# ilpoviertola/V-AURA

Hardware: AMD Instinct MI355X
Metric: audio codec tokens/sec (whole node), 2.56 s clips (higher is better)
Workload: dtype f16x2-split(22b)/f32-acc

## Files before the change

### vaura_amd/csrc/conv_kernels.h

```cpp
#pragma once
#include "common.h"

#define BM 128
#define BN 96
#define BK 32

struct ConvArgs {
  const float* in;
  const float* w;
  const float* bias;
  const float* res;
  const float* alpha;
  float* out_raw;
  float* out_act;
  int Lin, Lout, Cin, Cout, NT;
  int off_base, off_step;
  int ostride, oshift0;
  int jcount;
};

__host__ __device__ __forceinline__ size_t mx8_scale_offset(size_t elems) { return (elems + 15) & ~(size_t)15; }

__device__ __forceinline__ float snake_sin2(float x) {
  const float n = __builtin_rintf(x * 0.318309886183790672f);
  float r = fmaf(-n, 3.14159274101257324f, x);
  r = fmaf(-n, -8.74227765734758577e-8f, r);
  const float t = r * r;
  float p = fmaf(t, 2.6051661734527443e-06f, -0.00019809046352747828f);
  p = fmaf(t, p, 0.008333050645887852f);
  p = fmaf(t, p, -0.16666658222675323f);
  const float sn = fmaf(r, t * p, r);
  return sn * sn;
}
__device__ __forceinline__ float snake_fi(float v, float al, float inv) { return v + inv * snake_sin2(al * v); }
__device__ __forceinline__ float snake_f(float v, float al) { return snake_fi(v, al, 1.0f / (al + 1e-9f)); }

typedef _Float16 f16x8 __attribute__((ext_vector_type(8)));

struct ConvPArgs {
  const uint16_t* in;
  const uint16_t* w;
  const float* bias;
  const float* res;
  const float* alpha;
  float* out_raw;
  uint16_t* out_act;
  int Lin, Lout, Cin, Cout, NT;
  int off_base, off_step, ostride, oshift0, jcount;
  int act;
  int act_fmt;
  uint8_t* out_scale;
  const uint32_t* in_scale;
  const float* wscale;
  const uint16_t* w2;
  const float* bias2;
  const float* alpha_mid;
};

template <class Args>
static inline int va_conv_geometry(Args& a, int taps, int dilation, int stride, int Lin) {
  if (stride > 1) {
    a.NT = 2; a.off_base = 0; a.off_step = -1; a.ostride = stride; a.oshift0 = -(stride / 2);
    a.Lout = Lin * stride; a.jcount = Lin + 1;
    return stride;
  }
  a.NT = taps; a.off_base = -((taps - 1) / 2) * dilation; a.off_step = dilation;
  a.ostride = 1; a.oshift0 = 0; a.Lout = Lin; a.jcount = Lin;
  return 1;
}

int va_launch_conv_pair_tile(const ConvPArgs& p, int B, hipStream_t s);

__device__ __forceinline__ float gelu_erf_f(float x) {
  const float t = fabsf(x) * 0.70710678118654752440f;
  const float k = __builtin_amdgcn_rcpf(fmaf(t, 0.35f, 1.0f));
  float p = 0.06797561794519424f;
  p = fmaf(p, k, -0.4044332206249237f);
  p = fmaf(p, k, 0.8392713069915771f);
  p = fmaf(p, k, -0.7225478887557983f);
  p = fmaf(p, k, 0.6403822898864746f);
  p = fmaf(p, k, -0.046077974140644073f);
  p = fmaf(p, k, 0.23748238384723663f);
  p = fmaf(p, k, 0.1900186985731125f);
  p = fmaf(p, k, 0.1979287713766098f);
  const float e = (k * p) * __builtin_amdgcn_exp2f(-(t * t) * 1.4426950408889634f);
  return (0.5f * x) * (x < 0.f ? e : 2.0f - e);
}

__device__ __forceinline__ void store_pair4(uint16_t* base, size_t row, int c0, int C, const f32x4 v) {
  _Float16 h[4], l[4];
#pragma unroll
  for (int i = 0; i < 4; ++i) {
    const float x = v[i];
    h[i] = (_Float16)x;
    l[i] = (_Float16)(x - (float)h[i]);
  }
  typedef _Float16 f16x4 __attribute__((ext_vector_type(4)));
  f16x4* p = reinterpret_cast<f16x4*>(base + ((row * (size_t)(C >> 3) + (size_t)(c0 >> 3)) * 2) * 8 + (c0 & 7));
  p[0] = f16x4{h[0], h[1], h[2], h[3]};
  p[2] = f16x4{l[0], l[1], l[2], l[3]};
}

__device__ __forceinline__ int mx8_scale_byte(float amax) {
  const uint32_t bits = __builtin_bit_cast(uint32_t, amax);
  const int ea = (int)((bits >> 23) & 0xffu);
  const int e8 = ea - ((bits & 0x7fffffu) <= 0x600000u ? 8 : 7);
  return e8 < 1 ? 1 : (e8 > 253 ? 253 : e8);
}

__device__ __forceinline__ void store_act_octet(void* out_act, uint8_t* out_scale, int fmt, size_t grow, int co, int C,
                                                const float (&sv)[8]) {
  if (fmt == 0) {
    f16x8 hi, lo;
#pragma unroll
    for (int r = 0; r < 8; ++r) { hi[r] = (_Float16)sv[r]; lo[r] = (_Float16)(sv[r] - (float)hi[r]); }
    f16x8* dst = reinterpret_cast<f16x8*>(reinterpret_cast<uint16_t*>(out_act) + ((grow * (size_t)(C >> 3) + (size_t)(co >> 3)) * 2) * 8);
    dst[0] = hi;
    dst[1] = lo;
  } else {
    float amax = 0.f;
#pragma unroll
    for (int r = 0; r < 8; ++r) amax = fmaxf(amax, fabsf(sv[r]));
    amax = fmaxf(amax, __shfl_xor(amax, 1, 64));
    amax = fmaxf(amax, __shfl_xor(amax, 2, 64));
    const int e8 = mx8_scale_byte(amax);
    const float inv = __builtin_bit_cast(float, (uint32_t)(254 - e8) << 23);
    int q0 = 0, q1 = 0;
    q0 = __builtin_amdgcn_cvt_pk_fp8_f32(sv[0] * inv, sv[1] * inv, q0, false);
    q0 = __builtin_amdgcn_cvt_pk_fp8_f32(sv[2] * inv, sv[3] * inv, q0, true);
    q1 = __builtin_amdgcn_cvt_pk_fp8_f32(sv[4] * inv, sv[5] * inv, q1, false);
    q1 = __builtin_amdgcn_cvt_pk_fp8_f32(sv[6] * inv, sv[7] * inv, q1, true);
    typedef int i32x2 __attribute__((ext_vector_type(2)));
    *reinterpret_cast<i32x2*>(reinterpret_cast<uint8_t*>(out_act) + grow * (size_t)C + co) = i32x2{q0, q1};
    if (((co >> 3) & 3) == 0) out_scale[(grow * (size_t)((C + 127) >> 7) + (co >> 7)) * 4 + ((co >> 5) & 3)] = (uint8_t)e8;
  }
}

__device__ __forceinline__ float snake_fast(float v, float al) {
  const float sn = __builtin_amdgcn_sinf(__builtin_amdgcn_fractf(al * v * 0.15915494309189535f));
  return v + __builtin_amdgcn_rcpf(al + 1e-9f) * (sn * sn);
}

template <int BN_, int SP, bool FAST = false, int ROWS = BM>
__device__ __forceinline__ void conv_tile_store(const ConvPArgs& a, const float* stage, int b, int ph, int j0, int n0, int tid) {
  constexpr int OCT = BN_ / 8;
  static_assert(OCT % 4 == 0, "a 32-channel scale block = 4 consecutive threads of one row");
  constexpr int RSTEP = 256 / OCT;
  if (tid >= RSTEP * OCT) return;
  const int oc = tid % OCT, row0 = tid / OCT;
  const int co = n0 + oc * 8;
  const size_t obase = (size_t)b * a.Lout;
  f32x4 al0 = f32x4{0.f, 0.f, 0.f, 0.f}, al1 = al0, iv0 = al0, iv1 = al0;
  if (a.out_act && a.act == 0) {
    al0 = *reinterpret_cast<const f32x4*>(a.alpha + co);
    al1 = *reinterpret_cast<const f32x4*>(a.alpha + co + 4);
// ... 37 lines not shown
```

### vaura_amd/csrc/dac.hip

```cpp
#include "conv_kernels.h"
#include "dac_clips.h"

__global__ __launch_bounds__(256) void conv_mfma_kernel(ConvArgs a) {
  __shared__ f32x4 Ws[2][BK / 4][BN + 1];
  __shared__ f32x4 Xs[2][BK / 4][BM + 1];
  const int tid = threadIdx.x, lane = tid & 63, wv = tid >> 6;
  const int wn = wv & 1, wm = wv >> 1;
  const int j0 = blockIdx.x * BM;
  const int n0 = blockIdx.y * BN;
  const int tiles_m = gridDim.x;
  (void)tiles_m;
  const int phases = a.ostride;
  const int b = blockIdx.z / phases, ph = blockIdx.z % phases;
  const float* in = a.in + (size_t)b * a.Lin * a.Cin;
  const float* wbase = a.w + (size_t)ph * a.NT * a.Cout * a.Cin;
  const int kc = a.Cin / BK;
  const int nk = a.NT * kc;

  f32x4 wreg[3], xreg[4];
  auto load_tile = [&](int kt) {
    const int t = kt / kc, ci0 = (kt % kc) * BK;
    const float* wt = wbase + (size_t)t * a.Cout * a.Cin;
    const int off = a.off_base + t * a.off_step;
#pragma unroll
    for (int i = 0; i < 3; ++i) {
      const int qd = tid + 256 * i, row = qd >> 3, kq = qd & 7;
      wreg[i] = *reinterpret_cast<const f32x4*>(wt + (size_t)(n0 + row) * a.Cin + ci0 + 4 * kq);
    }
#pragma unroll
    for (int i = 0; i < 4; ++i) {
      const int qd = tid + 256 * i, row = qd >> 3, kq = qd & 7;
      const int jr = j0 + row + off;
      xreg[i] = (jr >= 0 && jr < a.Lin) ? *reinterpret_cast<const f32x4*>(in + (size_t)jr * a.Cin + ci0 + 4 * kq)
                                        : f32x4{0.f, 0.f, 0.f, 0.f};
    }
  };
  auto store_tile = [&](int buf) {
#pragma unroll
    for (int i = 0; i < 3; ++i) { const int qd = tid + 256 * i; Ws[buf][qd & 7][qd >> 3] = wreg[i]; }
#pragma unroll
    for (int i = 0; i < 4; ++i) { const int qd = tid + 256 * i; Xs[buf][qd & 7][qd >> 3] = xreg[i]; }
  };

  f32x4 acc[3][4];
#pragma unroll
  for (int i = 0; i < 3; ++i)
#pragma unroll
    for (int j = 0; j < 4; ++j) acc[i][j] = f32x4{0.f, 0.f, 0.f, 0.f};

  load_tile(0);
  store_tile(0);
  __syncthreads();
  for (int kt = 0; kt < nk; ++kt) {
    const int buf = kt & 1;
    if (kt + 1 < nk) load_tile(kt + 1);
#pragma unroll
    for (int c = 0; c < 2; ++c) {
      f32x4 af[3], bf[4];
#pragma unroll
      for (int i = 0; i < 3; ++i) af[i] = Ws[buf][4 * c + (lane >> 4)][wn * 48 + i * 16 + (lane & 15)];
#pragma unroll
      for (int j = 0; j < 4; ++j) bf[j] = Xs[buf][4 * c + (lane >> 4)][wm * 64 + j * 16 + (lane & 15)];
#pragma unroll
      for (int s = 0; s < 4; ++s)
#pragma unroll
        for (int i = 0; i < 3; ++i)
#pragma unroll
          for (int j = 0; j < 4; ++j)
            acc[i][j] = __builtin_amdgcn_mfma_f32_16x16x4f32(af[i][s], bf[j][s], acc[i][j], 0, 0, 0);
    }
    if (kt + 1 < nk) store_tile(buf ^ 1);
    __syncthreads();
  }

  const size_t obase = (size_t)b * a.Lout * a.Cout;
#pragma unroll
  for (int j = 0; j < 4; ++j) {
    const int jr = j0 + wm * 64 + j * 16 + (lane & 15);
    if (jr >= a.jcount) continue;
    const int orow = jr * a.ostride + a.oshift0 + ph;
    if (orow < 0 || orow >= a.Lout) continue;
#pragma unroll
    for (int i = 0; i < 3; ++i) {
      const int co = n0 + wn * 48 + i * 16 + 4 * (lane >> 4);
      const size_t o = obase + (size_t)orow * a.Cout + co;
      f32x4 v = acc[i][j] + *reinterpret_cast<const f32x4*>(a.bias + co);
      if (a.res) v = *reinterpret_cast<const f32x4*>(a.res + o) + v;
      if (a.out_raw) *reinterpret_cast<f32x4*>(a.out_raw + o) = v;
      if (a.out_act) {
        const f32x4 al = *reinterpret_cast<const f32x4*>(a.alpha + co);
        f32x4 s;
#pragma unroll
        for (int r = 0; r < 4; ++r) s[r] = snake_f(v[r], al[r]);
        *reinterpret_cast<f32x4*>(a.out_act + o) = s;
      }
    }
  }
}

#define XHALO 56
#define XROWS (BM + XHALO)
template <int NI, bool WS, bool XS = false, int MJ = 4, bool FUSE = false>
__global__ __launch_bounds__(256, 2) void conv_pair_kernel(ConvPArgs a) {
  constexpr int BN_ = 32 * NI;
  constexpr int BMT = 32 * MJ;
  constexpr int XROWS_T = BMT + XHALO;
  constexpr int NXB = MJ == 4 ? 2 : 1;
  static_assert(MJ == 4 || MJ == 8, "128 or 256 rows");
  constexpr int WSTR = (BN_ + 3 + 15) / 16 * 16, XSTR = (XROWS_T + 3 + 15) / 16 * 16;
  constexpr int WS_ELEMS = 2 * (BK / 4) * WSTR, XS_ELEMS = NXB * (BK / 4) * XSTR;
  constexpr int SP = BN_ + 4;
  static_assert((WS_ELEMS + XS_ELEMS) * 16 >= BM * SP * 4, "the output tile must fit in the main loop's LDS");
  static_assert(!FUSE || (NI == 3 && MJ == 8), "the fused residual unit: all 96 channels in one 256-row workgroup");
  constexpr int W1STR = 112, YSTR = 80;
  constexpr int W1_ELEMS = FUSE ? 3 * (BK / 4) * W1STR : 0, Y_ELEMS = FUSE ? 3 * (BK / 4) * YSTR : 0;
  static_assert(!FUSE || Y_ELEMS * 16 >= 64 * SP * 4, "the 64-row output tile is staged over the activated tile");
  constexpr int SMEM_ELEMS = (WS_ELEMS + XS_ELEMS) > (W1_ELEMS + Y_ELEMS) ? (WS_ELEMS + XS_ELEMS) : (W1_ELEMS + Y_ELEMS);
  constexpr int TAB_ELEMS = FUSE ? 2 * BN_ / 4 : 0;
  __shared__ u32x4 smem[SMEM_ELEMS + TAB_ELEMS];
  auto coff = [](int kq) { return (kq & 1) + ((kq >> 2) << 1); };
  auto Ws = [&](int buf, int kq, int row) -> u32x4& { return smem[(buf * (BK / 4) + kq) * WSTR + row + coff(kq)]; };
  auto Xs = [&](int buf, int kq, int row) -> u32x4& { return smem[WS_ELEMS + (buf * (BK / 4) + kq) * XSTR + row + coff(kq)]; };
  const int tid = threadIdx.x, lane = tid & 63, wv = tid >> 6;
  const int wn = wv & 1, wm = wv >> 1;
  const int j0 = blockIdx.x * BMT;
  const int n0 = blockIdx.y * BN_;
  const int phases = a.ostride;
  const int b = blockIdx.z / phases, ph = blockIdx.z % phases;
  const int cq = a.Cin / 4;
  const u32x4* in = reinterpret_cast<const u32x4*>(a.in) + (size_t)b * a.Lin * cq;
  const u32x4* wbase = reinterpret_cast<const u32x4*>(a.w) + (size_t)ph * a.NT * a.Cout * cq;
  const int kc = a.Cin / BK;
  const int NT = a.NT;
  const int nk = NT * kc;
  const int span = (NT - 1) * (a.off_step < 0 ? -a.off_step : a.off_step);
  const int lo_off = a.off_base + (a.off_step < 0 ? (NT - 1) * a.off_step : 0);
  const int xrows = BMT + span;
  constexpr int XL = (XROWS_T * (BK / 4) + 255) / 256;

  u32x4 wreg[NI], xreg[XL];
  auto load_w = [&](int kt) {
    const int c = kt / NT, t = kt - c * NT;
    const u32x4* wt = wbase + (size_t)t * a.Cout * cq;
    const int q0 = c * (BK / 4);
#pragma unroll
    for (int i = 0; i < NI; ++i) {
      const int qd = tid + 256 * i, row = qd >> 3, kq = qd & 7;
      wreg[i] = wt[(size_t)(n0 + row) * cq + q0 + kq];
    }
  };
  auto store_w = [&](int buf) {
#pragma unroll
    for (int i = 0; i < NI; ++i) { const int qd = tid + 256 * i; Ws(buf, qd & 7, qd >> 3) = wreg[i]; }
  };
  auto load_x = [&](int c) {
    const int q0 = c * (BK / 4);
#pragma unroll
    for (int i = 0; i < XL; ++i) {
      const int qd = tid + 256 * i, row = qd >> 3, kq = qd & 7;
      const int jr = j0 + lo_off + row;
      xreg[i] = (row < xrows && jr >= 0 && jr < a.Lin) ? in[(size_t)jr * cq + q0 + kq] : u32x4{0u, 0u, 0u, 0u};
    }
  };
  auto store_x = [&](int buf) {
#pragma unroll
    for (int i = 0; i < XL; ++i) {
      const int qd = tid + 256 * i;
      if ((qd >> 3) < XROWS_T) Xs(buf, qd & 7, qd >> 3) = xreg[i];
    }
  };

  f32x4 acc[NI][MJ];
#pragma unroll
  for (int i = 0; i < NI; ++i)
#pragma unroll
    for (int j = 0; j < MJ; ++j) acc[i][j] = f32x4{0.f, 0.f, 0.f, 0.f};

  VA_STAMP_DECL(stamps);
  VA_STAMP(stamps, 0);
  load_w(0);
  load_x(0);
  store_w(0);
  store_x(0);
  if constexpr (FUSE) {
    if (tid < BN_) {
      float* tab = reinterpret_cast<float*>(smem + SMEM_ELEMS);
      const float al = a.alpha_mid[tid];
      tab[tid] = al;
      tab[BN_ + tid] = 1.0f / (al + 1e-9f);
    }
  }
  __syncthreads();
  VA_STAMP(stamps, 1);
  const int g = lane >> 4, r16 = lane & 15;
  int kt = 0;
  for (int c = 0; c < kc; ++c) {
    const int xb = NXB == 2 ? (c & 1) : 0;
    for (int t = 0; t < NT; ++t, ++kt) {
      const int buf = kt & 1;
      if (kt + 1 < nk) load_w(kt + 1);
      if (t == (NXB == 2 ? 0 : NT - 1) && c + 1 < kc) load_x(c + 1);
      const int shift = a.off_base + t * a.off_step - lo_off;
      f16x8 wh[NI], wl[NI];
#pragma unroll
      for (int i = 0; i < NI; ++i) {
        wh[i] = __builtin_bit_cast(f16x8, Ws(buf, 2 * g, wn * (NI * 16) + i * 16 + r16));
        if constexpr (!WS && !XS) wl[i] = __builtin_bit_cast(f16x8, Ws(buf, 2 * g + 1, wn * (NI * 16) + i * 16 + r16));
      }
      constexpr int JG = MJ == 4 ? 4 : 2;
#pragma unroll
      for (int jh = 0; jh < MJ; jh += JG) {
        f16x8 xh[JG], xl[JG];
#pragma unroll
        for (int j = 0; j < JG; ++j) {
          xh[j] = __builtin_bit_cast(f16x8, Xs(xb, 2 * g, shift + wm * (16 * MJ) + (jh + j) * 16 + r16));
          if constexpr (!XS) xl[j] = __builtin_bit_cast(f16x8, Xs(xb, 2 * g + 1, shift + wm * (16 * MJ) + (jh + j) * 16 + r16));
        }
#pragma unroll
        for (int i = 0; i < NI; ++i)
#pragma unroll
          for (int j = 0; j < JG; ++j) {
            if constexpr (!WS && !XS) acc[i][jh + j] = __builtin_amdgcn_mfma_f32_16x16x32_f16(wl[i], xh[j], acc[i][jh + j], 0, 0, 0);
            if constexpr (!XS) acc[i][jh + j] = __builtin_amdgcn_mfma_f32_16x16x32_f16(wh[i], xl[j], acc[i][jh + j], 0, 0, 0);
            acc[i][jh + j] = __builtin_amdgcn_mfma_f32_16x16x32_f16(wh[i], xh[j], acc[i][jh + j], 0, 0, 0);
          }
      }
      if (kt + 1 < nk) store_w(buf ^ 1);
      if (t == NT - 1 && c + 1 < kc) {
        if constexpr (NXB == 1) __syncthreads();
        store_x(NXB == 2 ? (xb ^ 1) : 0);
      }
      __syncthreads();
    }
  }

  VA_STAMP(stamps, 2);
  if constexpr (FUSE) {
    u32x4* W1 = smem;
    u32x4* Yi = smem + W1_ELEMS;
    auto W1s = [&](int c2, int kq, int row) -> u32x4& { return W1[(c2 * (BK / 4) + kq) * W1STR + row + coff(kq)]; };
    auto Ys = [&](int c2, int kq, int row) -> u32x4& { return Yi[(c2 * (BK / 4) + kq) * YSTR + row + coff(kq)]; };
    u32x4 w1reg[9];
#pragma unroll
    for (int i = 0; i < 9; ++i) w1reg[i] = reinterpret_cast<const u32x4*>(a.w2)[tid + 256 * i];
    float* stage = reinterpret_cast<float*>(Yi);
    const float* tab = reinterpret_cast<const float*>(smem + SMEM_ELEMS);
    typedef _Float16 f16x4 __attribute__((ext_vector_type(4)));
    auto pass = [&](auto pc) {
      constexpr int p = decltype(pc)::value;
      if (p > 0) __syncthreads();
      if (wm == (p >> 1)) {
#pragma unroll
        for (int jj = 0; jj < 4; ++jj)
#pragma unroll
          for (int i = 0; i < NI; ++i) {
            const int col = wn * (NI * 16) + i * 16 + 4 * g;
            const f32x4 v = acc[i][4 * (p & 1) + jj] + *reinterpret_cast<const f32x4*>(a.bias + col);
            const f32x4 al = *reinterpret_cast<const f32x4*>(tab + col), iv = *reinterpret_cast<const f32x4*>(tab + BN_ + col);
            f16x4 h4, l4;
#pragma unroll
            for (int e = 0; e < 4; ++e) {
              const float sv = snake_fi(v[e], al[e], iv[e]);
              h4[e] = (_Float16)sv;
              l4[e] = (_Float16)(sv - (float)h4[e]);
            }
            const int c2 = col >> 5, o = (col & 31) >> 3, half = (col & 7) >> 2, row = jj * 16 + r16;
            reinterpret_cast<f16x4*>(&Ys(c2, 2 * o, row))[half] = h4;
            reinterpret_cast<f16x4*>(&Ys(c2, 2 * o + 1, row))[half] = l4;
          }
      }
      if (p == 0) {
#pragma unroll
        for (int i = 0; i < 9; ++i) {
          const int qd = tid + 256 * i, n = qd / 24, q = qd - n * 24;
          W1s(q >> 3, q & 7, n) = w1reg[i];
        }
      }
      __syncthreads();
      if (p == 0) VA_STAMP(stamps, 3);
      f32x4 acc2[NI][2];
#pragma unroll
      for (int i = 0; i < NI; ++i)
#pragma unroll
        for (int j = 0; j < 2; ++j) acc2[i][j] = f32x4{0.f, 0.f, 0.f, 0.f};
#pragma unroll
      for (int c2 = 0; c2 < 3; ++c2) {
        f16x8 wh[NI], wl[NI], xh[2], xl[2];
#pragma unroll
        for (int i = 0; i < NI; ++i) {
          wh[i] = __builtin_bit_cast(f16x8, W1s(c2, 2 * g, wn * (NI * 16) + i * 16 + r16));
          if constexpr (!WS && !XS) wl[i] = __builtin_bit_cast(f16x8, W1s(c2, 2 * g + 1, wn * (NI * 16) + i * 16 + r16));
        }
#pragma unroll
        for (int j = 0; j < 2; ++j) {
          xh[j] = __builtin_bit_cast(f16x8, Ys(c2, 2 * g, (wm * 2 + j) * 16 + r16));
          if constexpr (!XS) xl[j] = __builtin_bit_cast(f16x8, Ys(c2, 2 * g + 1, (wm * 2 + j) * 16 + r16));
        }
#pragma unroll
        for (int i = 0; i < NI; ++i)
#pragma unroll
          for (int j = 0; j < 2; ++j) {
            if constexpr (!WS && !XS) acc2[i][j] = __builtin_amdgcn_mfma_f32_16x16x32_f16(wl[i], xh[j], acc2[i][j], 0, 0, 0);
            if constexpr (!XS) acc2[i][j] = __builtin_amdgcn_mfma_f32_16x16x32_f16(wh[i], xl[j], acc2[i][j], 0, 0, 0);
            acc2[i][j] = __builtin_amdgcn_mfma_f32_16x16x32_f16(wh[i], xh[j], acc2[i][j], 0, 0, 0);
          }
      }
      __syncthreads();
      if (p == 0) VA_STAMP(stamps, 4);
#pragma unroll
      for (int i = 0; i < NI; ++i)
#pragma unroll
        for (int j = 0; j < 2; ++j) {
          const int row = (wm * 2 + j) * 16 + r16, col = wn * (NI * 16) + i * 16 + 4 * g;
          *reinterpret_cast<f32x4*>(stage + row * SP + col) = acc2[i][j] + *reinterpret_cast<const f32x4*>(a.bias2 + col);
        }
      __syncthreads();
// ... 484 lines not shown
  d += __shfl_xor(d, 1, 64);
  d += __shfl_xor(d, 2, 64);
  d += __shfl_xor(d, 4, 64);
  if (sub == 0 && l < L) wav[(size_t)b * L + l] = tanhf(d + bias[0]);
}

#define CO_TL 128
__global__ __launch_bounds__(256) void conv_out_tiled_kernel(const float* __restrict__ act, const float* __restrict__ w,
                                                              const float* __restrict__ bias, float* __restrict__ wav, int L, int C,
                                                              int pairs) {
  extern __shared__ __attribute__((aligned(16))) float rows[];
  const int b = blockIdx.y, l0 = blockIdx.x * CO_TL, tid = threadIdx.x;
  const int SR = C + 4, oct = C >> 3;
  for (int u = tid; u < (CO_TL + 6) * oct; u += 256) {
    const int rr = u / oct, oc = u - rr * oct;
    const int r = l0 - 3 + rr;
    float x[8];
    if (r < 0 || r >= L) {
#pragma unroll
      for (int e = 0; e < 8; ++e) x[e] = 0.f;
    } else if (pairs == 3) {
      const uint8_t* q = reinterpret_cast<const uint8_t*>(act) + (size_t)b * L * C;
      const int nsc = (C + 127) >> 7;
      const uint8_t* sc = reinterpret_cast<const uint8_t*>(act) + mx8_scale_offset((size_t)gridDim.y * L * C) + (size_t)b * L * nsc * 4;
      typedef int i32x2 __attribute__((ext_vector_type(2)));
      typedef float f32x2 __attribute__((ext_vector_type(2)));
      const i32x2 w8 = *reinterpret_cast<const i32x2*>(q + (size_t)r * C + 8 * oc);
      const int e8 = sc[((size_t)r * nsc + (oc >> 4)) * 4 + ((oc >> 2) & 3)];
      const float scl = __builtin_bit_cast(float, (uint32_t)e8 << 23);
      const f32x2 a0 = __builtin_amdgcn_cvt_pk_f32_fp8(w8.x, false), a1 = __builtin_amdgcn_cvt_pk_f32_fp8(w8.x, true);
      const f32x2 a2 = __builtin_amdgcn_cvt_pk_f32_fp8(w8.y, false), a3 = __builtin_amdgcn_cvt_pk_f32_fp8(w8.y, true);
      x[0] = a0.x * scl; x[1] = a0.y * scl; x[2] = a1.x * scl; x[3] = a1.y * scl;
      x[4] = a2.x * scl; x[5] = a2.y * scl; x[6] = a3.x * scl; x[7] = a3.y * scl;
    } else if (pairs) {
      const f16x8* pp = reinterpret_cast<const f16x8*>(reinterpret_cast<const _Float16*>(act) + (((size_t)b * L + r) * oct + oc) * 16);
      const f16x8 h = pp[0], lo = pp[1];
#pragma unroll
      for (int e = 0; e < 8; ++e) x[e] = (float)h[e] + (float)lo[e];
    } else {
      const f32x4* pp = reinterpret_cast<const f32x4*>(act + ((size_t)b * L + r) * C + 8 * oc);
      const f32x4 a0 = pp[0], a1 = pp[1];
      x[0] = a0[0]; x[1] = a0[1]; x[2] = a0[2]; x[3] = a0[3]; x[4] = a1[0]; x[5] = a1[1]; x[6] = a1[2]; x[7] = a1[3];
    }
    *reinterpret_cast<f32x4*>(rows + rr * SR + 8 * oc) = f32x4{x[0], x[1], x[2], x[3]};
    *reinterpret_cast<f32x4*>(rows + rr * SR + 8 * oc + 4) = f32x4{x[4], x[5], x[6], x[7]};
  }
  __syncthreads();
  const int half = __builtin_amdgcn_readfirstlane(tid >> 7), lo_ = tid & 127;
  const int c0 = half * (C >> 1), c1 = c0 + (C >> 1);
  f32x4 d4 = f32x4{0.f, 0.f, 0.f, 0.f};
#pragma unroll
  for (int t = 0; t < 7; ++t) {
    const f32x4* xr = reinterpret_cast<const f32x4*>(rows + (lo_ + t) * SR + c0);
    const f32x4* wr = reinterpret_cast<const f32x4*>(w + (size_t)t * C + c0);
#pragma unroll 4
    for (int c = 0; c < (c1 - c0) / 4; ++c) {
      const f32x4 x = xr[c], ww = wr[c];
      d4[0] = fmaf(x[0], ww[0], d4[0]); d4[1] = fmaf(x[1], ww[1], d4[1]); d4[2] = fmaf(x[2], ww[2], d4[2]); d4[3] = fmaf(x[3], ww[3], d4[3]);
    }
  }
  const float d = (d4[0] + d4[1]) + (d4[2] + d4[3]);
  float* part = rows + (CO_TL + 6) * SR;
  if (half) part[lo_] = d;
  __syncthreads();
  if (!half && l0 + lo_ < L) wav[(size_t)b * L + l0 + lo_] = tanhf((d + part[lo_]) + bias[0]);
}

__global__ __launch_bounds__(256) void act_convert_kernel(const float* __restrict__ in, void* out, uint8_t* out_scale, size_t rows,
                                                          int C, int fmt) {
  const size_t u = (size_t)blockIdx.x * 256 + threadIdx.x;
  const int oct = C >> 3;
  const size_t row = u / oct;
  if (row >= rows) return;
  const int co = (int)(u - row * oct) * 8;
  const f32x4 v0 = *reinterpret_cast<const f32x4*>(in + row * C + co), v1 = *reinterpret_cast<const f32x4*>(in + row * C + co + 4);
  const float sv[8] = {v0[0], v0[1], v0[2], v0[3], v1[0], v1[1], v1[2], v1[3]};
  store_act_octet(out, out_scale, fmt, row, co, C, sv);
}

static long long va_conv256_launches = 0;

typedef void (*ConvPairKernel)(ConvPArgs);
static ConvPairKernel conv_pair_instance(int ni, bool ws, bool xs, bool big) {
  if (ni == 3) {
    if (xs) return big ? conv_pair_kernel<3, true, true, 8> : conv_pair_kernel<3, true, true>;
    if (ws) return big ? conv_pair_kernel<3, true, false, 8> : conv_pair_kernel<3, true>;
    return big ? conv_pair_kernel<3, false, false, 8> : conv_pair_kernel<3, false>;
  }
  if (xs) return conv_pair_kernel<2, true, true>;
  if (ws) return big ? conv_pair_kernel<2, true, false, 8> : conv_pair_kernel<2, true>;
  return big ? conv_pair_kernel<2, false, false, 8> : conv_pair_kernel<2, false>;
}

static int launch_conv(const vaura_conv& cv, const float* in, const float* res, const float* alpha, float* out_raw,
                       float* out_act, int B, int Lin, int pairs, hipStream_t s) {
  if (!cv.w || !cv.bias || (cv.cin % BK)) return VAURA_ERR_SHAPE;
  if (out_act && !alpha) return VAURA_ERR_ARG;
  if (pairs) {
    if ((cv.cout % BN) && (cv.cout % 64)) return VAURA_ERR_SHAPE;
    ConvPArgs p;
    p.in = reinterpret_cast<const uint16_t*>(in); p.w = reinterpret_cast<const uint16_t*>(cv.w); p.bias = cv.bias; p.res = res;
    p.alpha = alpha; p.out_raw = out_raw; p.out_act = reinterpret_cast<uint16_t*>(out_act);
    p.Lin = Lin; p.Cin = cv.cin; p.Cout = cv.cout; p.act = 0;
    p.act_fmt = 0; p.out_scale = nullptr; p.in_scale = nullptr; p.wscale = nullptr;
    p.w2 = nullptr; p.bias2 = nullptr; p.alpha_mid = nullptr;
    if (cv.stride > 1 && (cv.stride % 2)) return VAURA_ERR_SHAPE;
    if (cv.stride <= 1 && (cv.taps - 1) * cv.dilation > XHALO) return VAURA_ERR_SHAPE;
    const int ph = va_conv_geometry(p, cv.taps, cv.dilation, cv.stride, Lin);
    if (pairs == 3) {
      if (out_act) {
        p.act_fmt = 1;
        p.out_scale = reinterpret_cast<uint8_t*>(out_act) + mx8_scale_offset((size_t)B * p.Lout * cv.cout);
      }
      if (cv.wscale) {
        if (cv.cout % BN) return VAURA_ERR_SHAPE;
        p.wscale = cv.wscale;
        p.in_scale = reinterpret_cast<const uint32_t*>(reinterpret_cast<const uint8_t*>(in) + mx8_scale_offset((size_t)B * Lin * cv.cin));
        VA_LAUNCH((conv_mx8_kernel<3>), dim3((p.jcount + BM - 1) / BM, cv.cout / BN, B * ph), dim3(256), 0, s, p);
        return 0;
      }
      pairs = 2;
    }
    const bool xs = pairs == 4, ws = xs || pairs == 2;
    const int ni = cv.cout % BN == 0 ? 3 : 2, tiles = cv.cout / (32 * ni);
    const int g256 = (p.jcount + 2 * BM - 1) / (2 * BM);
    const bool big = (ni == 3 || !xs) && !(va_debug_flags_get() & 0x100000u) && (int64_t)g256 * tiles * B * ph >= 384;
    if (big) ++va_conv256_launches;
    VA_LAUNCH(conv_pair_instance(ni, ws, xs, big), dim3(big ? g256 : (p.jcount + BM - 1) / BM, tiles, B * ph), dim3(256), 0, s, p);
    return 0;
  }
  if (cv.cout % BN) return VAURA_ERR_SHAPE;
  ConvArgs a;
  a.in = in; a.w = cv.w; a.bias = cv.bias; a.res = res; a.alpha = alpha; a.out_raw = out_raw; a.out_act = out_act;
  a.Lin = Lin; a.Cin = cv.cin; a.Cout = cv.cout;
  if (cv.stride > 1 && (cv.stride % 2)) return VAURA_ERR_SHAPE;
  const int phases = va_conv_geometry(a, cv.taps, cv.dilation, cv.stride, Lin);
  dim3 grid((a.jcount + BM - 1) / BM, cv.cout / BN, B * phases);
  VA_LAUNCH(conv_mfma_kernel, grid, dim3(256), 0, s, a);
  return 0;
}

int va_launch_conv_pair_tile(const ConvPArgs& p, int B, hipStream_t s) {
  VA_LAUNCH((conv_pair_kernel<3, false>), dim3((p.jcount + BM - 1) / BM, p.Cout / BN, B), dim3(256), 0, s, p);
  return 0;
}


#define VA_UNIT_NOT_ELIGIBLE (-0x7fffff00)
static long long va_conv_units_fused = 0;
static int launch_conv_unit(const vaura_conv& c7, const vaura_conv& c1, const float* in, const float* res, const float* alpha_mid,
                            const float* alpha_next, float* out_raw, float* out_act, int B, int L, int pairs, hipStream_t s) {
  if (pairs != 1 && pairs != 2 && pairs != 4) return VA_UNIT_NOT_ELIGIBLE;
  if (va_debug_flags_get() & (0x200000u | 0x100000u)) return VA_UNIT_NOT_ELIGIBLE;
  const int C = c7.cin;
  if ((C != BN && C != 2 * BN) || c7.cout != C || c1.cin != C || c1.cout != C || c7.stride != 1 || c1.stride != 1 || c1.taps != 1 || c7.taps < 1 ||
      (c7.taps - 1) * c7.dilation > XHALO || !c7.w || !c7.bias || !c1.w || !c1.bias || !alpha_mid || !alpha_next || !res || !out_act || (const float*)out_act == in)
    return VA_UNIT_NOT_ELIGIBLE;
  const int rows = C == BN ? 256 : 128;
  const int gx = (L + rows - 1) / rows;
  if ((int64_t)gx * B < 384) return VA_UNIT_NOT_ELIGIBLE;
  ConvPArgs p;
  p.in = reinterpret_cast<const uint16_t*>(in); p.w = reinterpret_cast<const uint16_t*>(c7.w); p.bias = c7.bias; p.res = res;
  p.alpha = alpha_next; p.out_raw = out_raw; p.out_act = reinterpret_cast<uint16_t*>(out_act);
  p.Lin = L; p.Cin = C; p.Cout = C; p.act = 0;
  p.act_fmt = 0; p.out_scale = nullptr; p.in_scale = nullptr; p.wscale = nullptr;
  va_conv_geometry(p, c7.taps, c7.dilation, 1, L);
  p.w2 = reinterpret_cast<const uint16_t*>(c1.w); p.bias2 = c1.bias; p.alpha_mid = alpha_mid;
  ++va_conv_units_fused;
  const dim3 grid(gx, 1, B);
  if (C == BN) {
    if (pairs == 4) VA_LAUNCH((conv_pair_kernel<3, true, true, 8, true>), grid, dim3(256), 0, s, p);
    else if (pairs == 2) VA_LAUNCH((conv_pair_kernel<3, true, false, 8, true>), grid, dim3(256), 0, s, p);
    else VA_LAUNCH((conv_pair_kernel<3, false, false, 8, true>), grid, dim3(256), 0, s, p);
  } else {
    if (pairs == 4) VA_LAUNCH((conv_unit_kernel<12, 2, true, true>), grid, dim3(256), 0, s, p);
    else if (pairs == 2) VA_LAUNCH((conv_unit_kernel<12, 2, true, false>), grid, dim3(256), 0, s, p);
    else VA_LAUNCH((conv_unit_kernel<12, 2, false, false>), grid, dim3(256), 0, s, p);
  }
  return 0;
}


VA_STAMP_SETTER(vaura_stamps_set_dac)

__global__ __launch_bounds__(256) void enc_conv_in_kernel(const float* __restrict__ wav, const float* __restrict__ w ,
                                                          const float* __restrict__ bias, const float* __restrict__ alpha,
                                                          float* __restrict__ out_raw, uint16_t* __restrict__ out_act, int64_t L,
                                                          int C) {
  const int b = blockIdx.y;
  const int qpr = C / 4;
  const int64_t gid = (int64_t)blockIdx.x * 256 + threadIdx.x;
  const int64_t l = gid / qpr;
  const int cq = (int)(gid % qpr);
  if (l >= L) return;
  const float* x = wav + (size_t)b * L;
  f32x4 v = *reinterpret_cast<const f32x4*>(bias + cq * 4);
#pragma unroll
  for (int t = 0; t < 7; ++t) {
    const int64_t r = l + t - 3;
    const float xv = (r >= 0 && r < L) ? x[r] : 0.f;
    v += *reinterpret_cast<const f32x4*>(w + t * C + cq * 4) * xv;
  }
  const size_t row = (size_t)b * L + (size_t)l;
  *reinterpret_cast<f32x4*>(out_raw + row * C + cq * 4) = v;
  const f32x4 al = *reinterpret_cast<const f32x4*>(alpha + cq * 4);
  f32x4 sn;
#pragma unroll
  for (int r = 0; r < 4; ++r) sn[r] = snake_f(v[r], al[r]);
  store_pair4(out_act, row, cq * 4, C, sn);
}

__global__ __launch_bounds__(256) void rvq_stage_kernel(float* __restrict__ residual ,
                                                        const float* __restrict__ in_w ,
                                                        const float* __restrict__ in_b, const float* __restrict__ cb ,
                                                        const float* __restrict__ out_w ,
                                                        const float* __restrict__ out_b, int32_t* __restrict__ codes, int latent,
                                                        int dim, int size, int T, int K, int k) {
  __shared__ float part[4][8];
  __shared__ float ze[8];
  __shared__ float bestv[4];
  __shared__ int besti[4];
  const int row = blockIdx.x, tid = threadIdx.x, lane = tid & 63, wv = tid >> 6;
  float* res = residual + (size_t)row * latent;
  float acc[8];
#pragma unroll
  for (int d = 0; d < 8; ++d) acc[d] = 0.f;
  for (int c = tid; c < latent; c += 256) {
    const float x = res[c];
#pragma unroll
    for (int d = 0; d < 8; ++d)
      if (d < dim) acc[d] = fmaf(in_w[(size_t)d * latent + c], x, acc[d]);
  }
#pragma unroll
  for (int d = 0; d < 8; ++d) {
    const float s = wave_sum(acc[d]);
    if (lane == 0) part[wv][d] = s;
  }
  __syncthreads();
  if (tid < 8) ze[tid] = tid < dim ? ((part[0][tid] + part[1][tid]) + (part[2][tid] + part[3][tid])) + in_b[tid] : 0.f;
  __syncthreads();
  float e[8], en2 = 0.f;
#pragma unroll
  for (int d = 0; d < 8; ++d) en2 = fmaf(ze[d], ze[d], en2);
  const float einv = 1.0f / fmaxf(sqrtf(en2), 1e-12f);
  float e2 = 0.f;
#pragma unroll
  for (int d = 0; d < 8; ++d) { e[d] = ze[d] * einv; e2 = fmaf(e[d], e[d], e2); }
  float bv = -INFINITY;
  int bi = 0x7fffffff;
  for (int j = tid; j < size; j += 256) {
    float c[8], cn2 = 0.f;
#pragma unroll
    for (int d = 0; d < 8; ++d) { c[d] = d < dim ? cb[(size_t)j * dim + d] : 0.f; cn2 = fmaf(c[d], c[d], cn2); }
    const float cinv = 1.0f / fmaxf(sqrtf(cn2), 1e-12f);
    float dot = 0.f, c2 = 0.f;
#pragma unroll
// ... 537 lines not shown
```

### vaura_amd/csrc/linear.hip

```cpp
#include "conv_kernels.h"

#define LBN 192
template <int MW>
__global__ __launch_bounds__(128 * MW, 2) void linear_pair_kernel(ConvPArgs a, int mtiles, int ntiles) {
  static_assert(MW == 2, "128 x 192 tiles");
  constexpr int NTH = 128 * MW, LBM_ = 64 * MW, NWQ = LBN * 8 / NTH, NXQ = LBM_ * 8 / NTH;
  __shared__ u32x4 smem[8 * (LBN + LBM_)];
  auto Ws = [&](int kq, int row) -> u32x4& { return smem[kq * LBN + (row ^ kq)]; };
  auto Xs = [&](int kq, int row) -> u32x4& { return smem[8 * LBN + kq * LBM_ + (row ^ kq)]; };
  const int tid = threadIdx.x, lane = tid & 63, wv = tid >> 6;
  const int wn = wv & 1, wm = wv >> 1;
  const int xcd = blockIdx.x & 7, local = blockIdx.x >> 3;
  const int nt = local % ntiles, mt = (local / ntiles) * 8 + xcd;
  if (mt >= mtiles) return;
  const int b = blockIdx.y;
  const int j0 = mt * LBM_, n0 = nt * LBN;
  const int cq = a.Cin / 4;
  const u32x4* in = reinterpret_cast<const u32x4*>(a.in) + (size_t)b * a.Lin * cq;
  const u32x4* wb = reinterpret_cast<const u32x4*>(a.w);
  const int nk = a.Cin / BK;

  u32x4 wreg[NWQ], xreg[NXQ];
  auto load_regs = [&](int kt) {
    const int q0 = kt * 8;
// ... 36 lines not shown
#pragma unroll
    for (int i = 0; i < 6; ++i) {
      const f16x8 wh = __builtin_bit_cast(f16x8, Ws(2 * g, wn * 96 + i * 16 + r16));
      const f16x8 wl = __builtin_bit_cast(f16x8, Ws(2 * g + 1, wn * 96 + i * 16 + r16));
#pragma unroll
      for (int j = 0; j < 4; ++j) {
        acc[i][j] = __builtin_amdgcn_mfma_f32_16x16x32_f16(wl, xh[j], acc[i][j], 0, 0, 0);
        acc[i][j] = __builtin_amdgcn_mfma_f32_16x16x32_f16(wh, xl[j], acc[i][j], 0, 0, 0);
        acc[i][j] = __builtin_amdgcn_mfma_f32_16x16x32_f16(wh, xh[j], acc[i][j], 0, 0, 0);
      }
    }
    __syncthreads();
  }

  constexpr int SP = LBN + 4, OCT = LBN / 8;
  static_assert(8 * (LBN + LBM_) * 16 >= 16 * MW * SP * 4, "the staged slab must fit in the main loop's LDS");
  float* stage = reinterpret_cast<float*>(smem);
  const size_t obase = (size_t)b * a.Lout;
#pragma unroll
  for (int j = 0; j < 4; ++j) {
#pragma unroll
    for (int i = 0; i < 6; ++i) {
      const int col = wn * 96 + i * 16 + 4 * g;
      *reinterpret_cast<f32x4*>(stage + (wm * 16 + r16) * SP + col) = acc[i][j] + *reinterpret_cast<const f32x4*>(a.bias + n0 + col);
    }
    __syncthreads();
#pragma unroll
    for (int it = 0; it < 16 * MW * OCT / NTH; ++it) {
      const int u = tid + NTH * it, lr = u / OCT, oc = u - lr * OCT;
      const int jr = j0 + (lr >> 4) * 64 + j * 16 + (lr & 15);
      if (jr < a.Lin) {
        const int co = n0 + oc * 8;
        const size_t orow = obase + (size_t)(jr + a.oshift0);
        const size_t o = orow * a.Cout + co;
        f32x4 v0 = *reinterpret_cast<const f32x4*>(stage + lr * SP + oc * 8);
        f32x4 v1 = *reinterpret_cast<const f32x4*>(stage + lr * SP + oc * 8 + 4);
        if (a.res) {
          v0 = *reinterpret_cast<const f32x4*>(a.res + o) + v0;
          v1 = *reinterpret_cast<const f32x4*>(a.res + o + 4) + v1;
        }
        if (a.out_raw) {
          *reinterpret_cast<f32x4*>(a.out_raw + o) = v0;
          *reinterpret_cast<f32x4*>(a.out_raw + o + 4) = v1;
        }
        if (a.out_act) {
          float sv[8];
#pragma unroll
          for (int r = 0; r < 4; ++r) {
            sv[r] = a.act == 1 ? gelu_erf_f(v0[r]) : v0[r];
            sv[r + 4] = a.act == 1 ? gelu_erf_f(v1[r]) : v1[r];
          }
          store_act_octet(a.out_act, nullptr, 0, orow, co, a.Cout, sv);
        }
      }
    }
    __syncthreads();
  }
}

template <int NST, int MW = 2, int NWN = 2, bool EARLY = false>
__global__ __launch_bounds__(64 * MW * NWN, (NST == 2 && MW * NWN == 4) ? 2 : 1) void linear_dma_kernel(ConvPArgs a, int mtiles, int ntiles, int panel) {
  static_assert(!EARLY || NST == 2, "EARLY is the two-stage schedule");
  typedef _Float16 f16x4 __attribute__((ext_vector_type(4)));
  typedef uint32_t u32x2 __attribute__((ext_vector_type(2)));
  constexpr int LBM_ = 64 * MW, NWV = NWN * MW, NI = 12 / NWN, WC = NI * 16, XF = (LBM_ / 16) * 2, WF = (LBN / 16) * 2, PPW = (XF + WF) / NWV, STB = (XF + WF) * 1024;
  static_assert((XF + WF) % NWV == 0, "the same number of pieces per wave");
  extern __shared__ __attribute__((aligned(16))) unsigned char lind_lds[];
  const int tid = threadIdx.x, lane = tid & 63;
  const int wv = __builtin_amdgcn_readfirstlane(tid >> 6);
  const int wn = wv % NWN, wm = wv / NWN;
  const int xcd = blockIdx.x & 7, local = blockIdx.x >> 3;
  const int rows_x = (mtiles + 7) >> 3, per_panel = rows_x * panel;
  const int pn = local / per_panel, lp = local - pn * per_panel;
  const int nt = pn * panel + lp % panel, mt = (lp / panel) * 8 + xcd;
  if (mt >= mtiles) return;
  const int b = blockIdx.y;
  const int j0 = mt * LBM_, n0 = nt * LBN;
  const int cq = a.Cin / 4;
  const int nk = a.Cin / BK;
  const int g = lane >> 4, r16 = lane & 15;

  const unsigned char* src[PPW];
  {
    const int k = lane >> 3, kk = k & 3;
    const int rr = (k >> 2) * 16 + 4 * (kk >> 1) + 8 * (kk & 1);
#pragma unroll
    for (int j = 0; j < PPW; ++j) {
      const int P = wv * PPW + j, pp = P & 3;
      const int q = ((lane & 7) - (pp + (pp >> 1) * 2)) & 7;
      if (P < XF) {
        const int row = min(j0 + (P >> 2) * 32 + rr + pp, a.Lin - 1);
        src[j] = reinterpret_cast<const unsigned char*>(a.in) + (((size_t)b * a.Lin + row) * cq + q) * 16;
      } else {
        src[j] = reinterpret_cast<const unsigned char*>(a.w) + ((size_t)(n0 + ((P - XF) >> 2) * 32 + rr + pp) * cq + q) * 16;
      }
    }
  }
  auto issue = [&](int stage) {
#pragma unroll
    for (int j = 0; j < PPW; ++j) {
      const int p = wv * PPW + j;
      __builtin_amdgcn_global_load_lds((const __attribute__((address_space(1))) void*)src[j],
                                       (__attribute__((address_space(3))) void*)(lind_lds + stage * STB + p * 1024), 16, 0, 0);
      src[j] += 128;
    }
  };
  int foff[2];
  {
    const int pp = r16 & 3, sp = pp + (pp >> 1) * 2, kq = (((r16 >> 3) & 1) + 2 * ((r16 >> 2) & 1)) * 8;
    foff[0] = pp * 1024 + (kq + ((2 * g + sp) & 7)) * 16;
    foff[1] = pp * 1024 + (kq + ((2 * g + 1 + sp) & 7)) * 16;
  }
  auto xfrag = [&](int stage, int m, int pl) -> f16x8 {
    return __builtin_bit_cast(f16x8, *reinterpret_cast<const u32x4*>(lind_lds + stage * STB + (m >> 1) * 4096 + (m & 1) * 512 + foff[pl]));
  };
  auto wfrag = [&](int stage, int n, int pl) -> f16x8 {
    return __builtin_bit_cast(f16x8, *reinterpret_cast<const u32x4*>(lind_lds + stage * STB + XF * 1024 + (n >> 1) * 4096 + (n & 1) * 512 + foff[pl]));
  };

  f32x4 acc[NI][4];
#pragma unroll
  for (int i = 0; i < NI; ++i)
#pragma unroll
    for (int j = 0; j < 4; ++j) acc[i][j] = f32x4{0.f, 0.f, 0.f, 0.f};

  if constexpr (EARLY) {
    issue(0);
    if (nk > 1) issue(1);
    for (int kt = 0; kt < nk; ++kt) {
      const int st = kt & 1;
      if (kt + 1 < nk) asm volatile("s_waitcnt vmcnt(%0)" ::"n"(PPW) : "memory");
      else asm volatile("s_waitcnt vmcnt(0)" ::: "memory");
      __builtin_amdgcn_s_barrier();
      asm volatile("" ::: "memory");
      f16x8 xh[4], xl[4], wh[NI], wl[NI];
#pragma unroll
      for (int j = 0; j < 4; ++j) {
        xh[j] = xfrag(st, wm * 4 + j, 0);
        xl[j] = xfrag(st, wm * 4 + j, 1);
      }
#pragma unroll
      for (int i = 0; i < NI; ++i) {
        wh[i] = wfrag(st, wn * NI + i, 0);
        wl[i] = wfrag(st, wn * NI + i, 1);
      }
      asm volatile("s_waitcnt lgkmcnt(0)" ::: "memory");
      __builtin_amdgcn_s_barrier();
      asm volatile("" ::: "memory");
      if (kt + 2 < nk) issue(st);
#pragma unroll
      for (int i = 0; i < NI; ++i)
#pragma unroll
        for (int j = 0; j < 4; ++j) {
          acc[i][j] = __builtin_amdgcn_mfma_f32_16x16x32_f16(wl[i], xh[j], acc[i][j], 0, 0, 0);
          acc[i][j] = __builtin_amdgcn_mfma_f32_16x16x32_f16(wh[i], xl[j], acc[i][j], 0, 0, 0);
          acc[i][j] = __builtin_amdgcn_mfma_f32_16x16x32_f16(wh[i], xh[j], acc[i][j], 0, 0, 0);
        }
    }
  } else {
#pragma unroll
  for (int st = 0; st < NST - 1; ++st)
    if (st < nk) issue(st);
  int st0 = 0;
  for (int kt = 0; kt < nk; ++kt) {
    {
      const int ahead = min(NST - 2, nk - 1 - kt);
      if (NST >= 4 && ahead >= 2) asm volatile("s_waitcnt vmcnt(%0)" ::"n"(2 * PPW) : "memory");
      else if (NST >= 3 && ahead == 1) asm volatile("s_waitcnt vmcnt(%0)" ::"n"(PPW) : "memory");
      else asm volatile("s_waitcnt vmcnt(0)" ::: "memory");
    }
    __builtin_amdgcn_s_barrier();
    asm volatile("" ::: "memory");
    if (kt + NST - 1 < nk) issue(st0 == 0 ? NST - 1 : st0 - 1);
    f16x8 xh[4], xl[4];
#pragma unroll
    for (int j = 0; j < 4; ++j) {
      xh[j] = xfrag(st0, wm * 4 + j, 0);
      xl[j] = xfrag(st0, wm * 4 + j, 1);
    }
#pragma unroll
    for (int i = 0; i < NI; ++i) {
      const f16x8 wh = wfrag(st0, wn * NI + i, 0);
      const f16x8 wl = wfrag(st0, wn * NI + i, 1);
#pragma unroll
      for (int j = 0; j < 4; ++j) {
        acc[i][j] = __builtin_amdgcn_mfma_f32_16x16x32_f16(wl, xh[j], acc[i][j], 0, 0, 0);
        acc[i][j] = __builtin_amdgcn_mfma_f32_16x16x32_f16(wh, xl[j], acc[i][j], 0, 0, 0);
        acc[i][j] = __builtin_amdgcn_mfma_f32_16x16x32_f16(wh, xh[j], acc[i][j], 0, 0, 0);
      }
    }
    st0 = st0 == NST - 1 ? 0 : st0 + 1;
  }
  }

  constexpr int SPW = WC + 4, QPR = WC / 4;
// ... 88 lines not shown
```

Baseline: 74120.

## Stream conv weights via LDS-DMA triple buffer in 256-row conv pair kernel

Adds a DMA variant of the 256-row conv pair kernel. Weight tiles are loaded straight into LDS with global_load_lds into a three-stage ring, instead of being staged through registers and written with store_w. The variant uses one barrier per k-step with explicit vmcnt waits. The goal is to cut the register pressure and VALU/LDS-store cost of weight staging and to overlap weight fetch with the MFMA work. The input tile still goes through registers and gets its own extra barrier at each restage. The new path is the default for the big and fused-unit launches, and a debug flag falls back to the old loop. Shared swizzle helpers are factored out of linear.hip.

```diff
diff --git a/vaura_amd/csrc/conv_kernels.h b/vaura_amd/csrc/conv_kernels.h
--- a/vaura_amd/csrc/conv_kernels.h
+++ b/vaura_amd/csrc/conv_kernels.h
@@ -71,6 +71,17 @@
 
 int va_launch_conv_pair_tile(const ConvPArgs& p, int B, hipStream_t s);
 
+__device__ __forceinline__ int va_dma_piece_row(int lane) {
+  const int k = lane >> 3, kk = k & 3;
+  return (k >> 2) * 16 + 4 * (kk >> 1) + 8 * (kk & 1);
+}
+__device__ __forceinline__ int va_dma_piece_quad(int lane, int pp) { return ((lane & 7) - (pp + (pp >> 1) * 2)) & 7; }
+__device__ __forceinline__ void va_dma_frag_off(int g, int r16, int (&foff)[2]) {
+  const int pp = r16 & 3, sp = pp + (pp >> 1) * 2, kq = (((r16 >> 3) & 1) + 2 * ((r16 >> 2) & 1)) * 8;
+  foff[0] = pp * 1024 + (kq + ((2 * g + sp) & 7)) * 16;
+  foff[1] = pp * 1024 + (kq + ((2 * g + 1 + sp) & 7)) * 16;
+}
+
 __device__ __forceinline__ float gelu_erf_f(float x) {
   const float t = fabsf(x) * 0.70710678118654752440f;
   const float k = __builtin_amdgcn_rcpf(fmaf(t, 0.35f, 1.0f));
diff --git a/vaura_amd/csrc/dac.hip b/vaura_amd/csrc/dac.hip
--- a/vaura_amd/csrc/dac.hip
+++ b/vaura_amd/csrc/dac.hip
@@ -100,15 +100,20 @@
 
 #define XHALO 56
 #define XROWS (BM + XHALO)
-template <int NI, bool WS, bool XS = false, int MJ = 4, bool FUSE = false>
+#define MJ_DMA (8 | 16)
+template <int NI, bool WS, bool XS = false, int MJ_ = 4, bool FUSE = false>
 __global__ __launch_bounds__(256, 2) void conv_pair_kernel(ConvPArgs a) {
+  constexpr int MJ = MJ_ & 15;
+  constexpr bool DMA = (MJ_ & 16) != 0;
   constexpr int BN_ = 32 * NI;
   constexpr int BMT = 32 * MJ;
   constexpr int XROWS_T = BMT + XHALO;
   constexpr int NXB = MJ == 4 ? 2 : 1;
   static_assert(MJ == 4 || MJ == 8, "128 or 256 rows");
+  static_assert(!DMA || MJ == 8, "the LDS-DMA loop is the 256-row one");
   constexpr int WSTR = (BN_ + 3 + 15) / 16 * 16, XSTR = (XROWS_T + 3 + 15) / 16 * 16;
-  constexpr int WS_ELEMS = 2 * (BK / 4) * WSTR, XS_ELEMS = NXB * (BK / 4) * XSTR;
+  constexpr int STB = BN_ * 128;
+  constexpr int WS_ELEMS = DMA ? 3 * STB / 16 : 2 * (BK / 4) * WSTR, XS_ELEMS = NXB * (BK / 4) * XSTR;
   constexpr int SP = BN_ + 4;
   static_assert((WS_ELEMS + XS_ELEMS) * 16 >= BM * SP * 4, "the output tile must fit in the main loop's LDS");
   static_assert(!FUSE || (NI == 3 && MJ == 8), "the fused residual unit: all 96 channels in one 256-row workgroup");
@@ -117,6 +122,7 @@
   static_assert(!FUSE || Y_ELEMS * 16 >= 64 * SP * 4, "the 64-row output tile is staged over the activated tile");
   constexpr int SMEM_ELEMS = (WS_ELEMS + XS_ELEMS) > (W1_ELEMS + Y_ELEMS) ? (WS_ELEMS + XS_ELEMS) : (W1_ELEMS + Y_ELEMS);
   constexpr int TAB_ELEMS = FUSE ? 2 * BN_ / 4 : 0;
+  static_assert(!DMA || (SMEM_ELEMS + TAB_ELEMS) * 16 <= 81920, "two workgroups share a CU's 160 KB");
   __shared__ u32x4 smem[SMEM_ELEMS + TAB_ELEMS];
   auto coff = [](int kq) { return (kq & 1) + ((kq >> 2) << 1); };
   auto Ws = [&](int buf, int kq, int row) -> u32x4& { return smem[(buf * (BK / 4) + kq) * WSTR + row + coff(kq)]; };
@@ -169,6 +175,29 @@
       if ((qd >> 3) < XROWS_T) Xs(buf, qd & 7, qd >> 3) = xreg[i];
     }
   };
+  constexpr int PPW = BN_ / 32;
+  const int wvu = __builtin_amdgcn_readfirstlane(wv);
+  unsigned char* const wlds = reinterpret_cast<unsigned char*>(smem);
+  const u32x4* wsrc[PPW];
+  int wfoff[2] = {0, 0};
+  if constexpr (DMA) {
+#pragma unroll
+    for (int j = 0; j < PPW; ++j) {
+      const int P = wvu * PPW + j, pp = P & 3;
+      wsrc[j] = wbase + (size_t)(n0 + (P >> 2) * 32 + va_dma_piece_row(lane) + pp) * cq + va_dma_piece_quad(lane, pp);
+    }
+    va_dma_frag_off(lane >> 4, lane & 15, wfoff);
+  }
+  int rq_c = 0, rq_t = 0, rq_st = 0;
+  auto issue_w = [&]() {
+    const size_t o = (size_t)rq_t * a.Cout * cq + (size_t)rq_c * (BK / 4);
+#pragma unroll
+    for (int j = 0; j < PPW; ++j)
+      __builtin_amdgcn_global_load_lds((const __attribute__((address_space(1))) void*)(wsrc[j] + o),
+                                       (__attribute__((address_space(3))) void*)(wlds + rq_st * STB + (wvu * PPW + j) * 1024), 16, 0, 0);
+    if (++rq_t == NT) { rq_t = 0; ++rq_c; }
+    rq_st = rq_st == 2 ? 0 : rq_st + 1;
+  };
 
   f32x4 acc[NI][MJ];
 #pragma unroll
@@ -178,10 +207,17 @@
 
   VA_STAMP_DECL(stamps);
   VA_STAMP(stamps, 0);
+  if constexpr (DMA) {
+    load_x(0);
+    issue_w();
+    if (nk > 1) issue_w();
+    store_x(0);
+  } else {
   load_w(0);
   load_x(0);
   store_w(0);
   store_x(0);
+  }
   if constexpr (FUSE) {
     if (tid < BN_) {
       float* tab = reinterpret_cast<float*>(smem + SMEM_ELEMS);
@@ -194,6 +230,55 @@
   VA_STAMP(stamps, 1);
   const int g = lane >> 4, r16 = lane & 15;
   int kt = 0;
+  if constexpr (DMA) {
+    int st = 0;
+    for (int c = 0; c < kc; ++c) {
+      for (int t = 0; t < NT; ++t, ++kt) {
+        if (kt + 1 < nk) asm volatile("s_waitcnt vmcnt(%0)" ::"n"(PPW) : "memory");
+        else asm volatile("s_waitcnt vmcnt(0)" ::: "memory");
+        asm volatile("s_waitcnt lgkmcnt(0)" ::: "memory");
+        __builtin_amdgcn_s_barrier();
+        asm volatile("" ::: "memory");
+        const bool restage = t == NT - 1 && c + 1 < kc;
+        if (restage) load_x(c + 1);
+        if (kt + 2 < nk) issue_w();
+        const int shift = a.off_base + t * a.off_step - lo_off;
+        const unsigned char* ws = wlds + st * STB;
+        f16x8 wh[NI], wl[NI];
+#pragma unroll
+        for (int i = 0; i < NI; ++i) {
+          const int n = wn * NI + i;
+          wh[i] = __builtin_bit_cast(f16x8, *reinterpret_cast<const u32x4*>(ws + (n >> 1) * 4096 + (n & 1) * 512 + wfoff[0]));
+          if constexpr (!WS && !XS) wl[i] = __builtin_bit_cast(f16x8, *reinterpret_cast<const u32x4*>(ws + (n >> 1) * 4096 + (n & 1) * 512 + wfoff[1]));
+        }
+#pragma unroll
+        for (int jh = 0; jh < MJ; jh += 2) {
+          f16x8 xh[2], xl[2];
+#pragma unroll
+          for (int j = 0; j < 2; ++j) {
+            xh[j] = __builtin_bit_cast(f16x8, Xs(0, 2 * g, shift + wm * (16 * MJ) + (jh + j) * 16 + r16));
+            if constexpr (!XS) xl[j] = __builtin_bit_cast(f16x8, Xs(0, 2 * g + 1, shift + wm * (16 * MJ) + (jh + j) * 16 + r16));
+          }
+#pragma unroll
+          for (int i = 0; i < NI; ++i)
+#pragma unroll
+            for (int j = 0; j < 2; ++j) {
+              if constexpr (!WS && !XS) acc[i][jh + j] = __builtin_amdgcn_mfma_f32_16x16x32_f16(wl[i], xh[j], acc[i][jh + j], 0, 0, 0);
+              if constexpr (!XS) acc[i][jh + j] = __builtin_amdgcn_mfma_f32_16x16x32_f16(wh[i], xl[j], acc[i][jh + j], 0, 0, 0);
+              acc[i][jh + j] = __builtin_amdgcn_mfma_f32_16x16x32_f16(wh[i], xh[j], acc[i][jh + j], 0, 0, 0);
+            }
+        }
+        if (restage) {
+          asm volatile("s_waitcnt lgkmcnt(0)" ::: "memory");
+          __builtin_amdgcn_s_barrier();
+          asm volatile("" ::: "memory");
+          store_x(0);
+        }
+        st = st == 2 ? 0 : st + 1;
+      }
+    }
+    __syncthreads();
+  } else {
   for (int c = 0; c < kc; ++c) {
     const int xb = NXB == 2 ? (c & 1) : 0;
     for (int t = 0; t < NT; ++t, ++kt) {
@@ -232,6 +317,7 @@
       }
       __syncthreads();
     }
+  }
   }
 
   VA_STAMP(stamps, 2);
@@ -882,6 +968,13 @@
 
 typedef void (*ConvPairKernel)(ConvPArgs);
 static ConvPairKernel conv_pair_instance(int ni, bool ws, bool xs, bool big) {
+  if (big && !(va_debug_flags_get() & 0x1000u)) {
+    if (ni == 3) {
+      if (xs) return conv_pair_kernel<3, true, true, MJ_DMA>;
+      return ws ? conv_pair_kernel<3, true, false, MJ_DMA> : conv_pair_kernel<3, false, false, MJ_DMA>;
+    }
+    return ws ? conv_pair_kernel<2, true, false, MJ_DMA> : conv_pair_kernel<2, false, false, MJ_DMA>;
+  }
   if (ni == 3) {
     if (xs) return big ? conv_pair_kernel<3, true, true, 8> : conv_pair_kernel<3, true, true>;
     if (ws) return big ? conv_pair_kernel<3, true, false, 8> : conv_pair_kernel<3, true>;
@@ -969,9 +1062,13 @@
   ++va_conv_units_fused;
   const dim3 grid(gx, 1, B);
   if (C == BN) {
-    if (pairs == 4) VA_LAUNCH((conv_pair_kernel<3, true, true, 8, true>), grid, dim3(256), 0, s, p);
-    else if (pairs == 2) VA_LAUNCH((conv_pair_kernel<3, true, false, 8, true>), grid, dim3(256), 0, s, p);
-    else VA_LAUNCH((conv_pair_kernel<3, false, false, 8, true>), grid, dim3(256), 0, s, p);
+    if (va_debug_flags_get() & 0x1000u) {
+      if (pairs == 4) VA_LAUNCH((conv_pair_kernel<3, true, true, 8, true>), grid, dim3(256), 0, s, p);
+      else if (pairs == 2) VA_LAUNCH((conv_pair_kernel<3, true, false, 8, true>), grid, dim3(256), 0, s, p);
+      else VA_LAUNCH((conv_pair_kernel<3, false, false, 8, true>), grid, dim3(256), 0, s, p);
+    } else if (pairs == 4) VA_LAUNCH((conv_pair_kernel<3, true, true, MJ_DMA, true>), grid, dim3(256), 0, s, p);
+    else if (pairs == 2) VA_LAUNCH((conv_pair_kernel<3, true, false, MJ_DMA, true>), grid, dim3(256), 0, s, p);
+    else VA_LAUNCH((conv_pair_kernel<3, false, false, MJ_DMA, true>), grid, dim3(256), 0, s, p);
   } else {
     if (pairs == 4) VA_LAUNCH((conv_unit_kernel<12, 2, true, true>), grid, dim3(256), 0, s, p);
     else if (pairs == 2) VA_LAUNCH((conv_unit_kernel<12, 2, true, false>), grid, dim3(256), 0, s, p);
diff --git a/vaura_amd/csrc/linear.hip b/vaura_amd/csrc/linear.hip
--- a/vaura_amd/csrc/linear.hip
+++ b/vaura_amd/csrc/linear.hip
@@ -142,12 +142,11 @@
 
   const unsigned char* src[PPW];
   {
-    const int k = lane >> 3, kk = k & 3;
-    const int rr = (k >> 2) * 16 + 4 * (kk >> 1) + 8 * (kk & 1);
+    const int rr = va_dma_piece_row(lane);
 #pragma unroll
     for (int j = 0; j < PPW; ++j) {
       const int P = wv * PPW + j, pp = P & 3;
-      const int q = ((lane & 7) - (pp + (pp >> 1) * 2)) & 7;
+      const int q = va_dma_piece_quad(lane, pp);
       if (P < XF) {
         const int row = min(j0 + (P >> 2) * 32 + rr + pp, a.Lin - 1);
         src[j] = reinterpret_cast<const unsigned char*>(a.in) + (((size_t)b * a.Lin + row) * cq + q) * 16;
@@ -166,11 +165,7 @@
     }
   };
   int foff[2];
-  {
-    const int pp = r16 & 3, sp = pp + (pp >> 1) * 2, kq = (((r16 >> 3) & 1) + 2 * ((r16 >> 2) & 1)) * 8;
-    foff[0] = pp * 1024 + (kq + ((2 * g + sp) & 7)) * 16;
-    foff[1] = pp * 1024 + (kq + ((2 * g + 1 + sp) & 7)) * 16;
-  }
+  va_dma_frag_off(g, r16, foff);
   auto xfrag = [&](int stage, int m, int pl) -> f16x8 {
     return __builtin_bit_cast(f16x8, *reinterpret_cast<const u32x4*>(lind_lds + stage * STB + (m >> 1) * 4096 + (m & 1) * 512 + foff[pl]));
   };
```

After: 74200, median of 2. No clear change (+0.1%).
